# curtischong/arreau

Measured on AMD Instinct MI355X. Metric: denoising steps/sec (crystal-steps, whole node), higher is better.
Workload: dtype f32

## Files before the change

### arreau_amd/csrc/edge_f16.hip

```cpp
#include <stdlib.h>
#include <utility>

#include "f16x3.h"
#define ARREAU_K_STORE_POLICY ""
#define ARREAU_K_STORE_TAIL "\n\ts_nop 3"
#include "internal.h"
#include "edge_rows.h"

#ifdef ARREAU_EDGE_TIMING
__device__ unsigned long long arreau_edge_ticks[8];
#define EDGE_TICK(i)                            \
    do {                                        \
        const long long now_ = clock64();       \
        tacc_[i] += now_ - tick_;               \
        tick_ = now_;                           \
    } while (0)
extern "C" int arreau_debug_edge_ticks(unsigned long long* out8, int reset) {
    if (hipMemcpyFromSymbol(out8, HIP_SYMBOL(arreau_edge_ticks), 64) != hipSuccess) return 1;
    if (reset) {
        unsigned long long z[8] = {0};
        if (hipMemcpyToSymbol(HIP_SYMBOL(arreau_edge_ticks), z, 64) != hipSuccess) return 1;
    }
    return 0;
}
#else
#define EDGE_TICK(i)
#endif

__device__ __forceinline__ unsigned round_lo_fp8(unsigned lo_pair) {
    typedef _Float16 h2_t __attribute__((ext_vector_type(2)));
    typedef short s2_t __attribute__((ext_vector_type(2)));
    s2_t r = {0, 0};
    r = __builtin_amdgcn_cvt_scalef32_pk_fp8_f16(r, __builtin_bit_cast(h2_t, lo_pair), 1.0f, false);
    return __builtin_bit_cast(unsigned, __builtin_amdgcn_cvt_scalef32_pk_f16_fp8(__builtin_bit_cast(unsigned, r), 1.0f, false));
}

__device__ __forceinline__ int relayout_cell(int plane, int row, int slot) { return 128 * plane + 4 * row + (slot ^ ((row >> 1) & 3)); }

template <int C, int D, int EH_WAVES, bool PROJ = true, bool BFP8 = false>
__global__ __launch_bounds__(64 * EH_WAVES, 2) void edge_kernel_f16x3(
    const float* __restrict__ nbr_dir,
    const float* __restrict__ nbr_dist,
    const int32_t* __restrict__ deg,
    const int32_t* __restrict__ batch,
    const float* __restrict__ lattice,
    const float* __restrict__ ori,
    const u32x4* __restrict__ stream,
    const float* __restrict__ b1, const float* __restrict__ b2, float r_max, int N, int k, int L,
    float* __restrict__ kbuf,
    int n0, int n1)
{
    constexpr int TC = C / 32, TD = D / 32, TM = ARREAU_MONO_PAD / 32;
    constexpr int NF1 = TM * 4, NF2 = TC * 4, NF3 = TD * 4;
    static_assert(TM == 3 && (TC & 1) == 0, "chunk geometry (projection tiles are walked in pairs)");
    __shared__ u32x4 lds[3][NF3 * 64];
    __shared__ __attribute__((aligned(16))) float otile[EH_WAVES][32 * 36];
    __shared__ __attribute__((aligned(16))) float bias_s[C + D];

    const int wave0 = __builtin_amdgcn_readfirstlane(threadIdx.x >> 6), lane0 = threadIdx.x & 63;
    const int npairs = (n1 - n0 + EH_WAVES / 4 - 1) / (EH_WAVES / 4);

#ifdef ARREAU_EDGE_TIMING
    long long tick_ = clock64();
    long long tacc_[8] = {0, 0, 0, 0, 0, 0, 0, 0};
    const long long c_start_ = tick_, w_start_ = wall_clock64();
#endif
    dma_chunk<NF1, EH_WAVES>(stream, lds[0], wave0, lane0);
    dma_chunk<NF1, EH_WAVES>(stream + (size_t)NF1 * 64, lds[1], wave0, lane0);
    if (threadIdx.x < C + D) bias_s[threadIdx.x] = threadIdx.x < C ? b1[threadIdx.x] : b2[threadIdx.x - C];
    int sl = 0;
    constexpr unsigned SLOT_BYTES = NF3 * 1024u;
    auto slot_after = [](int s_, int n) { const int r = s_ + n; return r >= 3 ? r - 3 : r; };
    const int nchunks = PROJ ? L * TC : 0;
    dma_wait();
    __syncthreads();
    int pend = 0;
    auto wait_copies = [&]() {
        if constexpr (PROJ) dma_wait();
        else {
            if (pend == 0) dma_wait();
            else if (pend == 2) dma_wait_but<2>();
            else dma_wait_but<4>();
        }
    };

    for (int pair = blockIdx.x; pair < npairs; pair += gridDim.x) {
        int lane = lane0, wave = wave0;
        asm volatile("" : "+v"(lane));
        asm volatile("" : "+s"(wave));
        const int h = lane >> 5, j = lane & 31;
        const int wn = wave & 3;
        const unsigned lane16 = 16u * lane;
        const unsigned lds0 = __builtin_amdgcn_readfirstlane((unsigned)(size_t)&lds[0][0]) + 1024u * wave;
        const bool has_next = pair + (int)gridDim.x < npairs;
        const int node_raw = n0 + (EH_WAVES / 4) * pair + (wave >> 2);
        const int node = min(node_raw, n1 - 1);
        const int nd = node_raw < n1 ? min(deg[node], k) : 0;
        const bool active = 2 * wn < nd;
        const u32x4* dma_src = stream + (size_t)2 * NF1 * 64;

        auto copy12 = [&](auto qtag) {
            constexpr int q2 = decltype(qtag)::value + 2;
            const int dst = slot_after(sl, 2);
            if constexpr (q2 < TC) {
                dma_chunk<NF1, EH_WAVES>(dma_src, lds[dst], wave, lane);
                dma_src += (size_t)NF1 * 64;
            } else if constexpr (q2 < TC + TD) {
                dma_chunk_lean<NF2, EH_WAVES>(dma_src, lane16, wave, lds0 + dst * SLOT_BYTES);
                dma_src += (size_t)NF2 * 64;
            } else if constexpr (PROJ) {
                dma_chunk_lean<NF3, EH_WAVES>(dma_src, lane16, wave, lds0 + dst * SLOT_BYTES);
                dma_src += (size_t)NF3 * 64;
            } else {
                if (has_next) dma_chunk<NF1, EH_WAVES>(stream + (size_t)(q2 - (TC + TD)) * NF1 * 64, lds[dst], wave, lane);
            }
            pend = 0;
        };
        auto copy3 = [&](int cidx) {
            const int dst = slot_after(sl, 2);
            if (cidx + 2 < nchunks) dma_chunk_lean<NF3, EH_WAVES>(dma_src, lane16, wave, lds0 + dst * SLOT_BYTES);
            else if (has_next)
                dma_chunk<NF1, EH_WAVES>(stream + (size_t)(cidx + 2 - nchunks) * NF1 * 64, lds[dst], wave, lane);
            dma_src += (size_t)NF3 * 64;
        };

        if (!active) {
            if constexpr (!PROJ) {
                if (node_raw < n1) {
                    constexpr unsigned SLOT = BFP8 ? 12288u : 16384u;
                    const char* blk = reinterpret_cast<const char*>(kbuf) + ((size_t)node * k + 2 * wn) * SLOT;
                    const u32x4 zero4 = {0u, 0u, 0u, 0u};
                    const int nblk = 2 * wn + 1 < k ? 2 : 1;
                    for (unsigned o = 0; o < (unsigned)nblk * SLOT; o += 1024u)
                        asm volatile("global_store_dwordx4 %0, %1, %2" ARREAU_K_STORE_TAIL : : "v"(lane16 + o), "v"(zero4), "s"(blk) : "memory");
                }
            }
            [&]<int... Q>(std::integer_sequence<int, Q...>) {
                ((dma_wait(), __syncthreads(), copy12(std::integral_constant<int, Q>{}), sl = slot_after(sl, 1)), ...);
            }(std::make_integer_sequence<int, TC + TD>{});
#pragma unroll 1
            for (int cidx = 0; cidx < nchunks; ++cidx) {
                dma_wait();
                __syncthreads();
                copy3(cidx);
                sl = slot_after(sl, 1);
            }
            EDGE_TICK(3);
            continue;
        }

        const int slot = 2 * wn + (j >> 4);
        const int o = j & 15;
        const int slot_c = min(slot, nd - 1);
        const float* Lm = lattice + 9 * (size_t)batch[node];
        const EdgeRow er = edge_row<true>(nbr_dir, nbr_dist, ori, Lm, (size_t)node * k + slot_c, o, r_max, slot < nd);
        const float window = er.window;
        Planes2 bm[TM];
        bm[0] = split_tile2(mono_tile<0>(er.a, h, std::make_integer_sequence<int, 16>{}));
        bm[1] = split_tile2(mono_tile<1>(er.a, h, std::make_integer_sequence<int, 16>{}));
        bm[2] = split_tile2(mono_tile<2>(er.a, h, std::make_integer_sequence<int, 16>{}));
        EDGE_TICK(0);

        int go = 1;
        asm volatile("" : "+s"(go));
        u32x4* pad16 = reinterpret_cast<u32x4*>(otile[wave]);
        const int c16 = lane & 15, g16 = lane >> 4;
        u32x4 h16[2][TC][2];
#pragma unroll
        for (int u = 0; u < TC; ++u)
#pragma unroll
            for (int nb = 0; nb < 2; ++nb) { h16[nb][u][0] = u32x4{0, 0, 0, 0}; h16[nb][u][1] = u32x4{0, 0, 0, 0}; }
        auto relayout_write = [&](const Planes2& pl) {
#pragma unroll
            for (int plane = 0; plane < 2; ++plane) {
                pad16[relayout_cell(plane, j, 2 * h + 0)] = pl.p[plane][0];
                pad16[relayout_cell(plane, j, 2 * h + 1)] = pl.p[plane][1];
            }
        };
        auto relayout_read = [&](int u) {
#pragma unroll
            for (int plane = 0; plane < 2; ++plane)
#pragma unroll
                for (int nb = 0; nb < 2; ++nb)
                    h16[nb][u][plane] = pad16[relayout_cell(plane, 16 * nb + c16, g16)];
        };
#pragma unroll
        for (int u = 0; u < TC; ++u) {
            f32x16 acc = arreau_bias_tile(bias_s, u, h), cross;
#pragma unroll
            for (int r = 0; r < 16; ++r) cross[r] = 0.f;
            MmaStream2<TM, 2 * TM> ms;
            ms.start(lds[sl], lane);
            if (go) ms.template run<0, TM>(acc, cross, bm);
            wait_copies();
            __syncthreads();
            if (u + 2 < TC) copy12(std::integral_constant<int, 0>{});
            else copy12(std::integral_constant<int, TC - 2>{});
            if (go) {
                ms.template run<TM, 2 * TM>(acc, cross, bm);
                const Planes2 pl = gelu_split_tile2(acc, cross, 1.0f);
                if (u > 0) relayout_read(u - 1);
                relayout_write(pl);
            }
            sl = slot_after(sl, 1);
        }
        relayout_read(TC - 1);
        float win16[2];
        win16[0] = __shfl(window, c16, 64);
        win16[1] = __shfl(window, 16 + c16, 64);
        EDGE_TICK(1);
        u32x4 b16[2][TD][2];
#pragma unroll
        for (int u = 0; u < TD; ++u) {
            Acc16 acc;
#pragma unroll
            for (int mt = 0; mt < 2; ++mt) {
                const f32x4 bv4 = *reinterpret_cast<const f32x4*>(bias_s + C + 32 * u + 16 * mt + 4 * g16);
#pragma unroll
                for (int nb = 0; nb < 2; ++nb) {
                    acc.m[mt][nb] = f32x4v{bv4[0], bv4[1], bv4[2], bv4[3]};
                    acc.x[mt][nb] = f32x4v{0.f, 0.f, 0.f, 0.f};
                }
            }
            MmaStream16<TC, true> ms;
            ms.start(lds[sl], lane);
            if (go) ms.template run<0, TC>(acc, h16);
            wait_copies();
            __syncthreads();
            if (u + 2 < TD) copy12(std::integral_constant<int, TC>{});
            else if constexpr (PROJ) copy12(std::integral_constant<int, TC + TD - 2>{});
            else if (u + 2 == TD) copy12(std::integral_constant<int, TC + TD - 2>{});
            else copy12(std::integral_constant<int, TC + TD - 1>{});
#pragma unroll
            for (int nb = 0; nb < 2; ++nb) { b16[nb][u][0] = u32x4{0, 0, 0, 0}; b16[nb][u][1] = u32x4{0, 0, 0, 0}; }
            if (go) {
                ms.template run<TC, 2 * TC>(acc, h16);
                unsigned lo8x[2][2] = {{0u, 0u}, {0u, 0u}};
#pragma unroll
                for (int nb = 0; nb < 2; ++nb) {
#pragma unroll
                    for (int mt = 0; mt < 2; ++mt)
#pragma unroll
                        for (int pr = 0; pr < 2; ++pr) {
                            const f32x2 pre = fma2(f32x2{acc.x[mt][nb][2 * pr], acc.x[mt][nb][2 * pr + 1]}, splat2(F16X3_INV_SCALE),
                                                   f32x2{acc.m[mt][nb][2 * pr], acc.m[mt][nb][2 * pr + 1]});
                            const f32x2 gw = gelu_fast2(pre) * splat2(win16[nb]);
                            unsigned hi, lo;
                            if constexpr (BFP8) {
                                if (pr == 0) split_pair_fp8<false>(gw, hi, lo8x[nb][mt]);
                                else split_pair_fp8<true>(gw, hi, lo8x[nb][mt]);
                                lo = pr == 0 ? widen_lo8<false>(lo8x[nb][mt]) : widen_lo8<true>(lo8x[nb][mt]);
                            } else {
                                split_pair2<false>(gw, hi, lo);
                            }
                            b16[nb][u][0][2 * mt + pr] = hi;
                            if constexpr (PROJ || !BFP8) b16[nb][u][1][2 * mt + pr] = lo;
                        }
                }
                if constexpr (!PROJ) {
                    const bool full_b = 2 * wn + 1 < k;
                    constexpr unsigned SLOT = BFP8 ? 12288u : 16384u;
                    const char* blk = reinterpret_cast<const char*>(kbuf) + ((size_t)node * k + 2 * wn) * SLOT;
#pragma unroll
                    for (int nb = 0; nb < 2; ++nb) {
                        if (nb == 1 && !full_b) continue;
                        if constexpr (BFP8) {
                            asm volatile("global_store_dwordx4 %0, %1, %2" ARREAU_K_STORE_TAIL
                                         :
                                         : "v"(lane16), "v"(b16[nb][u][0]), "s"(blk + SLOT * nb + 1024 * u)
                                         : "memory");
                            typedef unsigned u32x2_t __attribute__((ext_vector_type(2)));
                            const u32x2_t lo = {lo8x[nb][0], lo8x[nb][1]};
                            asm volatile("global_store_dwordx2 %0, %1, %2"
                                         :
                                         : "v"(lane16 >> 1), "v"(lo), "s"(blk + SLOT * nb + 8192 + 512 * u)
                                         : "memory");
                        } else {
#pragma unroll
                            for (int plane = 0; plane < 2; ++plane)
                                asm volatile("global_store_dwordx4 %0, %1, %2" ARREAU_K_STORE_TAIL
                                             :
                                             : "v"(lane16), "v"(b16[nb][u][plane]), "s"(blk + SLOT * nb + 2048 * u + 1024 * plane)
                                             : "memory");
                        }
                    }
                    pend += full_b ? 4 : 2;
                }
            }
            sl = slot_after(sl, 1);
        }
        EDGE_TICK(2);
        if constexpr (!PROJ) continue;
        const size_t layer_stride = (size_t)N * k * 16 * C;
        const size_t row0 = ((size_t)node * k + 2 * wn) * 16;
        const bool full = 2 * wn + 1 < k;
        const unsigned st_off = 4u * (c16 * C + 4 * g16);
        auto store_tile16 = [&](const Acc16& a, const char* tile_base ) {
#pragma unroll
            for (int nb = 0; nb < 2; ++nb)
#pragma unroll
                for (int mt = 0; mt < 2; ++mt) {
                    f32x4v v;
#pragma unroll
                    for (int r = 0; r < 4; ++r) v[r] = fmaf(a.x[mt][nb][r], F16X3_INV_SCALE, a.m[mt][nb][r]);
                    if (nb == 0 || full)
                        asm volatile("global_store_dwordx4 %0, %1, %2 offset:%3" ARREAU_K_STORE_POLICY ARREAU_K_STORE_TAIL
                                     :
                                     : "v"(st_off), "v"(v), "s"(tile_base + 64 * nb * C), "n"(64 * mt)
                                     : "memory");
                }
        };
        constexpr int ST = TD;
        const char* tile_base = reinterpret_cast<const char*>(kbuf) + row0 * C * 4;
        int u_cur = 0;
        Acc16 prev;
#pragma unroll
        for (int mt = 0; mt < 2; ++mt)
#pragma unroll
            for (int nb = 0; nb < 2; ++nb) { prev.m[mt][nb] = f32x4v{0.f, 0.f, 0.f, 0.f}; prev.x[mt][nb] = f32x4v{0.f, 0.f, 0.f, 0.f}; }
        auto chunk = [&](int cidx, Acc16& acc, const Acc16& prv) {
#pragma unroll
            for (int mt = 0; mt < 2; ++mt)
#pragma unroll
                for (int nb = 0; nb < 2; ++nb) { acc.m[mt][nb] = f32x4v{0.f, 0.f, 0.f, 0.f}; acc.x[mt][nb] = f32x4v{0.f, 0.f, 0.f, 0.f}; }
            MmaStream16<TD> ms;
            ms.start(lds[sl], lane);
            ms.template run<0, 2>(acc, b16);
            if (cidx > 0) {
                store_tile16(prv, tile_base);
                tile_base += (++u_cur == TC) ? (u_cur = 0, (ptrdiff_t)layer_stride * 4 - (TC - 1) * 32 * 4) : 32 * 4;
            }
            ms.template run<2, ST>(acc, b16);
            if (cidx == 0) dma_wait();
            else if (full) dma_wait_but<4>();
            else dma_wait_but<2>();
            __syncthreads();
            copy3(cidx);
            ms.template run<ST, 2 * TD>(acc, b16);
            sl = slot_after(sl, 1);
        };
        Acc16 accA;
#pragma unroll 1
        for (int cidx = 0; cidx < nchunks; cidx += 2) {
            chunk(cidx, accA, prev);
            chunk(cidx + 1, prev, accA);
        }
        store_tile16(prev, tile_base);
        EDGE_TICK(3);
    }
    dma_wait();
    EDGE_TICK(4);
#ifdef ARREAU_EDGE_TIMING
    tacc_[5] = clock64() - c_start_;
    tacc_[6] = wall_clock64() - w_start_;
    if (threadIdx.x == 0)
        for (int i = 0; i < 8; ++i) atomicAdd(&arreau_edge_ticks[i], (unsigned long long)tacc_[i]);
#endif
}

#define ARREAU_EDGE_SPLIT_MAX_NODES 240
template <int C, int D, bool BFP8>
__global__ __launch_bounds__(512) void edge_kernel_f16x3_split(
    const float* __restrict__ nbr_dir, const float* __restrict__ nbr_dist, const int32_t* __restrict__ deg,
    const int32_t* __restrict__ batch, const float* __restrict__ lattice, const float* __restrict__ ori,
    const u32x4* __restrict__ stream, const float* __restrict__ b1, const float* __restrict__ b2, float r_max, int N, int k,
    int L, float* __restrict__ kbuf, int n0) {
    constexpr int TC = C / 32, TD = D / 32, TM = ARREAU_MONO_PAD / 32;
    constexpr int NF1 = TM * 4, NF2 = TC * 4, NF3 = TD * 4;
    static_assert(TM == 3 && TC == 4 && TD == 8, "wave roles below assume C = 128, D = 256");
    __shared__ u32x4 hpad[TC][256];
    __shared__ u32x4 bpad[TD][2][2][64];

    const int wave = __builtin_amdgcn_readfirstlane(threadIdx.x >> 6), lane = threadIdx.x & 63;
    const int node = n0 + (int)(blockIdx.x >> 2), wn = blockIdx.x & 3;
    const int nd = min(deg[node], k);
    if (2 * wn >= nd) return;
    const int h = lane >> 5, j = lane & 31;
    const int c16 = lane & 15, g16 = lane >> 4;

    const u32x4* s1 = stream;
    const u32x4* s2 = stream + (size_t)TC * NF1 * 64;
    const u32x4* s3 = s2 + (size_t)TD * NF2 * 64;
    const int nchunks = L * TC;

    u32x4 w1[NF1], w2[NF2], wx[16], wy[16];
    if (wave < TC) {
#pragma unroll
        for (int i = 0; i < NF1; ++i) w1[i] = s1[(size_t)wave * NF1 * 64 + i * 64 + lane];
    }
#pragma unroll
    for (int i = 0; i < NF2; ++i) w2[i] = s2[(size_t)wave * NF2 * 64 + i * 64 + lane];
    auto load_half = [&](u32x4 (&w)[16], int cidx, int half) {
        const u32x4* src = s3 + (size_t)cidx * NF3 * 64 + (size_t)half * 16 * 64 + lane;
#pragma unroll
        for (int i = 0; i < 16; ++i) w[i] = src[i * 64];
    };

    const int slot = 2 * wn + (j >> 4);
    const int o = j & 15;
    const int slot_c = min(slot, nd - 1);
    const float* Lm = lattice + 9 * (size_t)batch[node];
    const EdgeRow er = edge_row<true>(nbr_dir, nbr_dist, ori, Lm, (size_t)node * k + slot_c, o, r_max, slot < nd);
    const float window = er.window;
    float win16[2];
    win16[0] = __shfl(window, c16, 64);
    win16[1] = __shfl(window, 16 + c16, 64);

    if (wave < TC) {
        Planes2 bm[TM];
        bm[0] = split_tile2(mono_tile<0>(er.a, h, std::make_integer_sequence<int, 16>{}));
        bm[1] = split_tile2(mono_tile<1>(er.a, h, std::make_integer_sequence<int, 16>{}));
        bm[2] = split_tile2(mono_tile<2>(er.a, h, std::make_integer_sequence<int, 16>{}));
        f32x16 acc = arreau_bias_tile(b1, wave, h), cross;
#pragma unroll
        for (int r = 0; r < 16; ++r) cross[r] = 0.f;
#pragma unroll
        for (int ks = 0; ks < 2 * TM; ++ks) {
            const int t = ks >> 1, s = ks & 1;
            acc = mfma_f16(w1[2 * ks], bm[t].p[0][s], acc);
            cross = mfma_f16(w1[2 * ks + 1], bm[t].p[0][s], cross);
            acc = mfma_f16(w1[2 * ks], bm[t].p[1][s], acc);
        }
        const Planes2 pl = gelu_split_tile2(acc, cross, 1.0f);
#pragma unroll
        for (int plane = 0; plane < 2; ++plane) {
            hpad[wave][relayout_cell(plane, j, 2 * h + 0)] = pl.p[plane][0];
            hpad[wave][relayout_cell(plane, j, 2 * h + 1)] = pl.p[plane][1];
        }
    }
    __syncthreads();
    asm volatile("" ::: "memory");
    load_half(wx, wave, 0);

    {
        Acc16 acc;
#pragma unroll
        for (int mt = 0; mt < 2; ++mt) {
            const f32x4 bv4 = *reinterpret_cast<const f32x4*>(b2 + 32 * wave + 16 * mt + 4 * g16);
#pragma unroll
            for (int nb = 0; nb < 2; ++nb) {
                acc.m[mt][nb] = f32x4v{bv4[0], bv4[1], bv4[2], bv4[3]};
                acc.x[mt][nb] = f32x4v{0.f, 0.f, 0.f, 0.f};
            }
        }
#pragma unroll
        for (int kb = 0; kb < TC; ++kb) {
            u32x4 hq[2][2];
#pragma unroll
            for (int nb = 0; nb < 2; ++nb)
#pragma unroll
                for (int plane = 0; plane < 2; ++plane)
                    hq[nb][plane] = hpad[kb][relayout_cell(plane, 16 * nb + c16, g16)];
#pragma unroll
            for (int mt = 0; mt < 2; ++mt)
#pragma unroll
                for (int nb = 0; nb < 2; ++nb) {
                    const int st = 2 * kb + mt;
                    acc.m[mt][nb] = mfma16_f16(w2[2 * st], hq[nb][0], acc.m[mt][nb]);
                    acc.x[mt][nb] = mfma16_f16(w2[2 * st + 1], hq[nb][0], acc.x[mt][nb]);
                    acc.m[mt][nb] = mfma16_f16(w2[2 * st], hq[nb][1], acc.m[mt][nb]);
                }
            __builtin_amdgcn_sched_barrier(0);
        }
#pragma unroll
        for (int nb = 0; nb < 2; ++nb) {
            u32x4 hi4, lo4;
#pragma unroll
            for (int mt = 0; mt < 2; ++mt)
#pragma unroll
                for (int pr = 0; pr < 2; ++pr) {
                    const f32x2 pre = fma2(f32x2{acc.x[mt][nb][2 * pr], acc.x[mt][nb][2 * pr + 1]}, splat2(F16X3_INV_SCALE),
                                           f32x2{acc.m[mt][nb][2 * pr], acc.m[mt][nb][2 * pr + 1]});
                    const f32x2 gw = gelu_fast2(pre) * splat2(win16[nb]);
                    unsigned hi, lo;
                    if constexpr (BFP8) {
                        unsigned l8 = 0u;
                        split_pair_fp8<false>(gw, hi, l8);
                        lo = widen_lo8<false>(l8);
                    } else {
                        split_pair2<false>(gw, hi, lo);
                    }
                    hi4[2 * mt + pr] = hi;
                    lo4[2 * mt + pr] = lo;
                }
            bpad[wave][nb][0][lane] = hi4;
            bpad[wave][nb][1][lane] = lo4;
        }
    }
    asm volatile("" ::: "memory");
    load_half(wy, wave, 1);
    __syncthreads();
    asm volatile("" ::: "memory");

    const size_t layer_stride = (size_t)N * k * 16 * C;
    const size_t row0 = ((size_t)node * k + 2 * wn) * 16;
    const bool full = 2 * wn + 1 < k;
    Acc16 acc;
    auto zero_acc = [&]() {
#pragma unroll
        for (int mt = 0; mt < 2; ++mt)
#pragma unroll
            for (int nb = 0; nb < 2; ++nb) { acc.m[mt][nb] = f32x4v{0.f, 0.f, 0.f, 0.f}; acc.x[mt][nb] = f32x4v{0.f, 0.f, 0.f, 0.f}; }
    };
    auto half_steps = [&](const u32x4 (&w)[16], int half) {
        u32x4 bq[2][4];
#pragma unroll
        for (int i = 0; i < 4; ++i) bq[0][i] = bpad[4 * half][i >> 1][i & 1][lane];
#pragma unroll
        for (int kbi = 0; kbi < 4; ++kbi) {
            if (kbi + 1 < 4) {
#pragma unroll
                for (int i = 0; i < 4; ++i) bq[(kbi + 1) & 1][i] = bpad[4 * half + kbi + 1][i >> 1][i & 1][lane];
            }
#pragma unroll
            for (int mt = 0; mt < 2; ++mt)
#pragma unroll
                for (int nb = 0; nb < 2; ++nb) {
                    const int i = 2 * kbi + mt;
                    acc.m[mt][nb] = mfma16_f16(w[2 * i], bq[kbi & 1][2 * nb], acc.m[mt][nb]);
                    acc.x[mt][nb] = mfma16_f16(w[2 * i], bq[kbi & 1][2 * nb + 1], acc.x[mt][nb]);
                    acc.x[mt][nb] = mfma16_f16(w[2 * i + 1], bq[kbi & 1][2 * nb], acc.x[mt][nb]);
                }
            __builtin_amdgcn_sched_barrier(0);
        }
    };
    auto store_tile = [&](int cidx) {
        const int l = cidx / TC, u = cidx % TC;
        float* tile = kbuf + (size_t)l * layer_stride + row0 * C + 32 * u;
#pragma unroll
        for (int nb = 0; nb < 2; ++nb)
#pragma unroll
            for (int mt = 0; mt < 2; ++mt) {
                f32x4 v;
#pragma unroll
                for (int r = 0; r < 4; ++r) v[r] = fmaf(acc.x[mt][nb][r], F16X3_INV_SCALE, acc.m[mt][nb][r]);
                if (nb == 0 || full) *reinterpret_cast<f32x4*>(tile + (size_t)(16 * nb + c16) * C + 16 * mt + 4 * g16) = v;
            }
    };
    zero_acc();
    half_steps(wx, 0);
    if (wave + 8 < nchunks) load_half(wx, wave + 8, 0);
    half_steps(wy, 1);
    store_tile(wave);
    if (wave + 8 < nchunks) {
        load_half(wy, wave + 8, 1);
        zero_acc();
        half_steps(wx, 0);
        if (wave + 16 < nchunks) load_half(wx, wave + 16, 0);
        half_steps(wy, 1);
        store_tile(wave + 8);
        if (wave + 16 < nchunks) {
            load_half(wy, wave + 16, 1);
            zero_acc();
            half_steps(wx, 0);
            half_steps(wy, 1);
            store_tile(wave + 16);
        }
    }
}

int arreau_launch_edge_f16x3(const arreau_model* m, const float* dir, const float* dist, const int32_t* deg,
                             const int32_t* batch, const float* lattice, int N, float* kbuf, hipStream_t s) {
    if (N <= 0) return ARREAU_OK;
    if (!(m->C == 128 && m->D == 256 && m->k <= 8)) {
        arreau_set_error("edge kernel (fp16x3): unsupported (hidden_dim, basis_dim, max_neighbors)");
        return ARREAU_EINVAL;
    }
    static const int wgs_env = [] { const char* e = getenv("ARREAU_EDGE_WGS"); return e ? atoi(e) : 0; }();
    static const int split_env = [] { const char* e = getenv("ARREAU_EDGE_SPLIT"); return e ? atoi(e) : -1; }();
    const bool split_ok = m->L * 4 >= 8 && m->L * 4 <= 24;
    const bool use_split = split_ok && !arreau_basis_form(m, N) &&
                           (split_env >= 0 ? split_env != 0 : N <= ARREAU_EDGE_SPLIT_MAX_NODES);
    if (use_split) {
        auto launch = [&](auto kernel) {
            ARREAU_LAUNCH(kernel, dim3((unsigned)N * 4), dim3(512), 0, s, dir, dist, deg, batch, lattice, m->ori,
                               reinterpret_cast<const u32x4*>(m->edge_f16), m->b1, m->b2, m->cfg.radius, N, m->k, m->L, kbuf, 0);
        };
        if (arreau_basis_fp8(m)) launch(edge_kernel_f16x3_split<128, 256, true>);
        else launch(edge_kernel_f16x3_split<128, 256, false>);
        ARREAU_CHECK_HIP(hipGetLastError());
        return ARREAU_OK;
    }
    const int npairs = (N + 1) / 2;
    const int n_cu = arreau_cu_count();
    const int wgs = wgs_env > 0 ? (wgs_env < npairs ? wgs_env : npairs) : (npairs < n_cu ? npairs : n_cu);
    if (arreau_basis_form(m, N)) {
        if (arreau_basis_fp8(m))
            ARREAU_LAUNCH((edge_kernel_f16x3<128, 256, 8, false, true>), dim3(wgs), dim3(512), 0, s, dir, dist, deg, batch, lattice, m->ori,
                          reinterpret_cast<const u32x4*>(m->edge_f16), m->b1, m->b2, m->cfg.radius, N, m->k, m->L, kbuf, 0, N);
        else
            ARREAU_LAUNCH((edge_kernel_f16x3<128, 256, 8, false, false>), dim3(wgs), dim3(512), 0, s, dir, dist, deg, batch, lattice, m->ori,
                          reinterpret_cast<const u32x4*>(m->edge_f16), m->b1, m->b2, m->cfg.radius, N, m->k, m->L, kbuf, 0, N);
        ARREAU_CHECK_HIP(hipGetLastError());
        return ARREAU_OK;
    }
    auto launch = [&](auto kernel) {
        ARREAU_LAUNCH(kernel, dim3(wgs), dim3(512), 0, s, dir, dist, deg, batch, lattice, m->ori,
                           reinterpret_cast<const u32x4*>(m->edge_f16), m->b1, m->b2, m->cfg.radius, N, m->k, m->L, kbuf, 0, N);
    };
    if (arreau_basis_fp8(m)) launch(edge_kernel_f16x3<128, 256, 8, true, true>);
    else launch(edge_kernel_f16x3<128, 256, 8, true, false>);
    ARREAU_CHECK_HIP(hipGetLastError());
    return ARREAU_OK;
}
```

Before: 192,200.

## Generalize edge kernel LDS weight ring to configurable prefetch depth

Makes the depth of the LDS weight-chunk ring configurable for the non-projection (basis) variant, so chunks are prefetched AHEAD = NSLOT-1 steps ahead instead of a fixed two. Pending-store accounting becomes a per-step array, letting wait_copies wait only for the oldest copies while younger copies and stores stay in flight. The default ring depth of 3 keeps the same schedule, except the tail copy of next-node chunks is now issued even when there is no next pair. Deeper rings would cost LDS and could lower occupancy.

```diff
diff --git a/arreau_amd/csrc/edge_f16.hip b/arreau_amd/csrc/edge_f16.hip
--- a/arreau_amd/csrc/edge_f16.hip
+++ b/arreau_amd/csrc/edge_f16.hip
@@ -6,6 +6,9 @@
 #define ARREAU_K_STORE_TAIL "\n\ts_nop 3"
 #include "internal.h"
 #include "edge_rows.h"
+#ifndef ARREAU_EDGE_BASIS_RING
+#define ARREAU_EDGE_BASIS_RING 3
+#endif
 
 #ifdef ARREAU_EDGE_TIMING
 __device__ unsigned long long arreau_edge_ticks[8];
@@ -53,7 +56,11 @@
     constexpr int TC = C / 32, TD = D / 32, TM = ARREAU_MONO_PAD / 32;
     constexpr int NF1 = TM * 4, NF2 = TC * 4, NF3 = TD * 4;
     static_assert(TM == 3 && (TC & 1) == 0, "chunk geometry (projection tiles are walked in pairs)");
-    __shared__ u32x4 lds[3][NF3 * 64];
+    constexpr int NSLOT = PROJ ? 3 : ARREAU_EDGE_BASIS_RING, AHEAD = NSLOT - 1;
+    constexpr int SLOT_FRAGS = PROJ ? NF3 : NF2;
+    static_assert(NSLOT >= 3 && AHEAD <= TC, "ring depth: the prologue copies layer-1 chunks only");
+    static_assert((NF1 + EH_WAVES - 1) / EH_WAVES == 2 && NF2 / EH_WAVES == 2, "two copy instructions per wave and chunk (wait_copies)");
+    __shared__ u32x4 lds[NSLOT][SLOT_FRAGS * 64];
     __shared__ __attribute__((aligned(16))) float otile[EH_WAVES][32 * 36];
     __shared__ __attribute__((aligned(16))) float bias_s[C + D];
 
@@ -65,23 +72,43 @@
     long long tacc_[8] = {0, 0, 0, 0, 0, 0, 0, 0};
     const long long c_start_ = tick_, w_start_ = wall_clock64();
 #endif
-    dma_chunk<NF1, EH_WAVES>(stream, lds[0], wave0, lane0);
-    dma_chunk<NF1, EH_WAVES>(stream + (size_t)NF1 * 64, lds[1], wave0, lane0);
+#pragma unroll
+    for (int q = 0; q < AHEAD; ++q) dma_chunk<NF1, EH_WAVES>(stream + (size_t)q * NF1 * 64, lds[q], wave0, lane0);
     if (threadIdx.x < C + D) bias_s[threadIdx.x] = threadIdx.x < C ? b1[threadIdx.x] : b2[threadIdx.x - C];
     int sl = 0;
-    constexpr unsigned SLOT_BYTES = NF3 * 1024u;
-    auto slot_after = [](int s_, int n) { const int r = s_ + n; return r >= 3 ? r - 3 : r; };
+    constexpr unsigned SLOT_BYTES = SLOT_FRAGS * 1024u;
+    auto slot_after = [](int s_, int n) { const int r = s_ + n; return r >= NSLOT ? r - NSLOT : r; };
     const int nchunks = PROJ ? L * TC : 0;
     dma_wait();
     __syncthreads();
-    int pend = 0;
+    int pend[AHEAD - 1];
+#pragma unroll
+    for (int i = 0; i < AHEAD - 1; ++i) pend[i] = 0;
     auto wait_copies = [&]() {
         if constexpr (PROJ) dma_wait();
         else {
-            if (pend == 0) dma_wait();
-            else if (pend == 2) dma_wait_but<2>();
-            else dma_wait_but<4>();
-        }
+            int young = 2 * (AHEAD - 2);
+#pragma unroll
+            for (int i = 0; i < AHEAD - 1; ++i) young += pend[i];
+            switch (young) {
+                case 2: dma_wait_but<2>(); break;
+                case 4: dma_wait_but<4>(); break;
+                case 6: dma_wait_but<6>(); break;
+                case 8: dma_wait_but<8>(); break;
+                case 10: dma_wait_but<10>(); break;
+                case 12: dma_wait_but<12>(); break;
+                case 14: dma_wait_but<14>(); break;
+                case 16: dma_wait_but<16>(); break;
+                case 18: dma_wait_but<18>(); break;
+                default: dma_wait();
+            }
+        }
+    };
+    auto stores_issued = [&](int n) { pend[0] += n; };
+    auto copies_issued = [&]() {
+#pragma unroll
+        for (int i = AHEAD - 2; i > 0; --i) pend[i] = pend[i - 1];
+        pend[0] = 0;
     };
 
     for (int pair = blockIdx.x; pair < npairs; pair += gridDim.x) {
@@ -97,24 +124,24 @@
         const int node = min(node_raw, n1 - 1);
         const int nd = node_raw < n1 ? min(deg[node], k) : 0;
         const bool active = 2 * wn < nd;
-        const u32x4* dma_src = stream + (size_t)2 * NF1 * 64;
+        const u32x4* dma_src = stream + (size_t)AHEAD * NF1 * 64;
 
         auto copy12 = [&](auto qtag) {
-            constexpr int q2 = decltype(qtag)::value + 2;
-            const int dst = slot_after(sl, 2);
-            if constexpr (q2 < TC) {
+            constexpr int qa = decltype(qtag)::value + AHEAD;
+            const int dst = slot_after(sl, AHEAD);
+            if constexpr (qa < TC) {
                 dma_chunk<NF1, EH_WAVES>(dma_src, lds[dst], wave, lane);
                 dma_src += (size_t)NF1 * 64;
-            } else if constexpr (q2 < TC + TD) {
+            } else if constexpr (qa < TC + TD) {
                 dma_chunk_lean<NF2, EH_WAVES>(dma_src, lane16, wave, lds0 + dst * SLOT_BYTES);
                 dma_src += (size_t)NF2 * 64;
             } else if constexpr (PROJ) {
                 dma_chunk_lean<NF3, EH_WAVES>(dma_src, lane16, wave, lds0 + dst * SLOT_BYTES);
                 dma_src += (size_t)NF3 * 64;
             } else {
-                if (has_next) dma_chunk<NF1, EH_WAVES>(stream + (size_t)(q2 - (TC + TD)) * NF1 * 64, lds[dst], wave, lane);
-            }
-            pend = 0;
+                dma_chunk<NF1, EH_WAVES>(stream + (size_t)(qa - (TC + TD)) * NF1 * 64, lds[dst], wave, lane);
+            }
+            copies_issued();
         };
         auto copy3 = [&](int cidx) {
             const int dst = slot_after(sl, 2);
@@ -194,8 +221,8 @@
             if (go) ms.template run<0, TM>(acc, cross, bm);
             wait_copies();
             __syncthreads();
-            if (u + 2 < TC) copy12(std::integral_constant<int, 0>{});
-            else copy12(std::integral_constant<int, TC - 2>{});
+            if (u + AHEAD < TC) copy12(std::integral_constant<int, 0>{});
+            else copy12(std::integral_constant<int, TC - 1>{});
             if (go) {
                 ms.template run<TM, 2 * TM>(acc, cross, bm);
                 const Planes2 pl = gelu_split_tile2(acc, cross, 1.0f);
@@ -227,10 +254,12 @@
             if (go) ms.template run<0, TC>(acc, h16);
             wait_copies();
             __syncthreads();
-            if (u + 2 < TD) copy12(std::integral_constant<int, TC>{});
+            if (u + AHEAD < TD) copy12(std::integral_constant<int, TC>{});
             else if constexpr (PROJ) copy12(std::integral_constant<int, TC + TD - 2>{});
-            else if (u + 2 == TD) copy12(std::integral_constant<int, TC + TD - 2>{});
-            else copy12(std::integral_constant<int, TC + TD - 1>{});
+            else
+                [&]<int... J>(std::integer_sequence<int, J...>) {
+                    ((u + AHEAD - TD == J ? copy12(std::integral_constant<int, TC + TD - AHEAD + J>{}) : void()), ...);
+                }(std::make_integer_sequence<int, AHEAD>{});
 #pragma unroll
             for (int nb = 0; nb < 2; ++nb) { b16[nb][u][0] = u32x4{0, 0, 0, 0}; b16[nb][u][1] = u32x4{0, 0, 0, 0}; }
             if (go) {
@@ -284,7 +313,7 @@
                                              : "memory");
                         }
                     }
-                    pend += full_b ? 4 : 2;
+                    stores_issued(full_b ? 4 : 2);
                 }
             }
             sl = slot_after(sl, 1);
```

After: 191,300. No clear change (-0.5%).
